# quocdat32461997/ggpm

Hardware: AMD Instinct MI355X
Metric: HierMPNEncoder fwd+bwd target row (SURVEY 8(d): encoder + KL heads + optimizer, tree fixed-point hint on; full depth loops in full_depth_loops, the full VAE fwd+bwd row in vae_step) of BASELINE's molecules/sec VAE fwd+bwd (hidden=300, depth=20, batch=32) (higher is better)
Workload: dtype f32

## Files before the change

### ggpm_amd/_lib.py

```python
from __future__ import annotations

import ctypes
import os
from ctypes import c_char_p, c_double, c_float, c_int, c_size_t, c_void_p, POINTER

from . import build as _build

_LIB = None

GGPM_OK, GGPM_ERR_ARG, GGPM_ERR_LAUNCH, GGPM_ERR_UNSUPPORTED, GGPM_ERR_WORKSPACE = range(5)

P = c_void_p
I = c_int
SIGNATURES = {
    "ggpm_version": (I, []),
    "ggpm_error_string": (c_char_p, [I]),
    "ggpm_padded_hidden": (I, [I]),
    "ggpm_padded_to_csr": (I, [P, I, I, P, P, P]),
    "ggpm_padded_to_csr_pair": (I, [P, I, I, P, P, P, I, I, P, P, P]),
    "ggpm_csr_transpose": (I, [P, P, I, I, P, P, P, P]),
    "ggpm_extract_column": (I, [P, I, I, I, P, P]),
    "ggpm_gemm_workspace_bytes": (c_size_t, [I, I, I]),
    "ggpm_gemm": (I, [I, I, I, I, I, P, I, P, I, P, I, I, P, I, I, I, P, c_size_t, P]),
    "ggpm_gemm_grouped": (I, [I, I, I, I, I, I, P, P]),
# ... 14 lines not shown
    "ggpm_gather_rows": (I, [P, I, P, I, I, P, I, I, I, P]),
    "ggpm_scatter_rows": (I, [P, I, P, I, I, P, I, I, P]),
    "ggpm_adam_step": (I, [P, P, P, P, c_size_t, c_float, c_float, c_float, c_float, c_float, I, P]),
    "ggpm_flat_sqnorm_workspace_bytes": (c_size_t, [c_size_t]),
    "ggpm_flat_sqnorm_partials": (I, [P, c_size_t, P, c_size_t, P]),
    "ggpm_flat_norm_finish": (I, [P, I, c_float, P, P]),
    "ggpm_adam_step_groups": (I, [P, P, P, P, c_size_t, P, I, P, I, P, I, c_float, P, I, P]),
    "ggpm_adam_step_ex": (I, [P, P, P, P, c_size_t, P, I, P, I, P, I, c_float, I, P, c_float, I, I, P, P, P, P]),
    "ggpm_flat_swap": (I, [P, P, c_size_t, P]),
    "ggpm_onehot": (I, [P, I, I, P, I, I, I, P]),
    "ggpm_embed_graph": (I, [P, I, P, I, I, I, I, P, I, P, I, P]),
    "ggpm_level_bf16_storage": (I, [I, I]),
    "ggpm_level_form_query": (I, [I, I, I, I, I, P, P]),
    "ggpm_level_q_part_bytes": (c_size_t, [I, I]),
    "ggpm_level_ksplit_q": (I, [I, I, I, I, P]),
    "ggpm_gru_backward_stashes": (I, [P, I, I, I, POINTER(c_void_p), POINTER(c_void_p)]),
    "ggpm_lstm_backward_stashes": (I, [P, I, I, I, POINTER(c_void_p), POINTER(c_void_p), POINTER(c_void_p)]),
    "ggpm_sum_slots": (I, [P, I, c_size_t, P, P]),
    "ggpm_gru_pack_floats": (c_size_t, [I]),
    "ggpm_gru_forward": (I, [I, I, I, P, P, P, P, I, P, I, P, P, I, P, P, P, P, P, P, P, P, P, P, I, P, P]),
    "ggpm_gru_backward_workspace_bytes": (c_size_t, [I, I, I]),
    "ggpm_gru_backward": (I, [I, I, I, P, P, I, P, I, P, I, P, P, P, P, P, P, P, P, P, P, P, P, P, P, P,
                              P, I, P, I, P, P, I, P, c_size_t, I, P, P]),
    "ggpm_gru_weight_grads": (I, [I, I, I, P, P, P, P, c_size_t, P, I, P, I, P, P, I, P, P]),
    "ggpm_gru_sparse_forward": (I, [I, I, I, P, P, P, P, P, P, I, P, I, P, P, I, P, P, P, P, P, P, P, P, P, P, I, P, P]),
    "ggpm_gru_sparse_backward": (I, [I, I, I, P, P, P, I, P, I, P, I, P, P, P, P, P, P, P, P, P, P, P, P, P, P, P, P,
                                     P, I, P, I, P, P, I, P, c_size_t, P, P]),
    "ggpm_weight_grads_stacked_workspace_bytes": (c_size_t, [I, I]),
    "ggpm_gru_weight_grads_stacked": (I, [I, I, I, P, P, P, P, P, P, P, I, P, I, P, P, I, P, c_size_t, P]),
    "ggpm_lstm_weight_grads_stacked": (I, [I, I, I, P, P, P, P, P, P, P, I, P, I, P, I, P, I, P, c_size_t, P]),
# ... 125 lines not shown
```

### ggpm_amd/csrc/encoder.hip

```cpp
#include "common.h"
#include "level_call.h"
#include <condition_variable>
#include <cstdlib>
#include <deque>
#include <functional>
#include <mutex>
#include <thread>

namespace {

struct Arena {
    char* base;
    size_t off;
    bool overflow;
    size_t cap;
    template <typename T>
    T* take(size_t n) {
        const size_t bytes = (n * sizeof(T) + 255) & ~(size_t)255;
        T* p = base ? reinterpret_cast<T*>(base + off) : nullptr;
        off += bytes;
        if (base && off > cap) overflow = true;
        return p;
    }
};
// ... 74 lines not shown
    const size_t slot = (size_t)E1 * Hp;
    L.X = A.take<float>(cell_gates(lstm).n * slot);
    L.Hs = A.take<float>((size_t)(depth + 1) * slot);
    L.Cs = lstm ? A.take<float>((size_t)(depth + 1) * slot) : nullptr;
    L.Qs = A.take<float>((size_t)depth * slot);
    L.St = A.take<float>((size_t)5 * depth * slot);
    L.wpack = A.take<float>(ggpm_level_pack_floats(lstm, H));
    L.nei = A.take<float>((size_t)N1 * Hp);
}

void take_q_part(Arena& A, const Dims& d, LevelSaved& L) {
    const ggpm_level_opts o = level_opts(d);
    L.qpart = nullptr; L.qpart_bytes = 0;
    if (!ggpm_level_ksplit_q(d.lstm, d.E1t, d.H, 0, &o)) return;
    L.qpart_bytes = ggpm_level_q_part_bytes(d.E1t, d.H);
    L.qpart = A.take<float>(L.qpart_bytes / sizeof(float));
}

void layout_saved(Arena& A, const Dims& d, Saved& s) {
    s.lv[0].hout = s.lv[1].hout = s.lv[2].hout = nullptr;
    take_csr(A, s.gpred, d.E1g, d.E1g, d.E1g * d.Kgb);
    take_csr(A, s.gagr, d.N1g, d.E1g, d.N1g * d.Kga);
    take_csr(A, s.tpred, d.E1t, d.E1t, d.E1t * d.Ktb);
    take_csr(A, s.tagr, d.N1t, d.E1t, d.N1t * d.Kta);
    take_csr(A, s.tcgr, d.N1t, d.N1g, d.N1t * d.Ktc);
    s.src = A.take<int32_t>(d.E1t); s.attr0 = A.take<int32_t>(d.E1t);
    s.motif_id = A.take<int32_t>(d.N1t); s.attach_id = A.take<int32_t>(d.N1t);
    const int nio = (d.E1t > d.N1t ? d.E1t : d.N1t) + 1;
    s.iota = A.take<int32_t>(nio > d.B + 1 ? nio : d.B + 1);
    auto take_index = [&](Csr& c, int rows, int ncols) {
// ... 4 lines not shown
    take_index(s.tsrc, d.E1t, d.N1t);
    take_index(s.root, d.B, d.N1t);
    take_index(s.motif, d.N1t, d.n_motif);
    take_index(s.attach, d.N1t, d.n_attach);
    s.hnode_a = A.take<float>((size_t)d.N1g * d.ld_n);
    s.hmess_a = A.take<float>((size_t)d.E1g * d.ld_m);
    take_level(A, s.lv[0], d.E1t, d.N1t, d.Hp, d.H, d.depthT, d.lstm);
    take_level(A, s.lv[1], d.E1t, d.N1t, d.Hp, d.H, d.depthT, d.lstm);
    take_level(A, s.lv[2], d.E1g, d.N1g, d.Hp, d.H, d.depthG, d.lstm);
    s.finput_i = A.take<float>((size_t)d.N1t * d.Hep); s.pooled = A.take<float>((size_t)d.N1t * d.Hp);
    s.hnode_i = A.take<float>((size_t)d.N1t * d.Hp); s.hmess_i = A.take<float>((size_t)d.E1t * d.ld_t);
    s.finput_t = A.take<float>((size_t)d.N1t * d.Hep);
    s.hnode_t = A.take<float>((size_t)d.N1t * d.Hp); s.hmess_t = A.take<float>((size_t)d.E1t * d.ld_t);
    s.f = A.take<float>((size_t)d.B * d.Hp); s.n = A.take<float>((size_t)d.B * d.Hp);
    for (int l = 0; l < 2; ++l) take_q_part(A, d, s.lv[l]);
    s.lv[2].qpart = nullptr; s.lv[2].qpart_bytes = 0;
}

void take_csr_fwd(Arena& A, Csr& c, int rows, int ncols, int cap) {
    c.rows = rows; c.ncols = ncols; c.cap = cap < 1 ? 1 : cap;
    c.rowptr = A.take<int32_t>(rows + 1);
    c.col = A.take<int32_t>(c.cap);
    c.rowptrT = c.colT = c.cursor = nullptr;
}

void layout_infer(Arena& A, const Dims& d, Saved& s) {
    s = Saved{};
    take_csr_fwd(A, s.gpred, d.E1g, d.E1g, d.E1g * d.Kgb);
    take_csr_fwd(A, s.gagr, d.N1g, d.E1g, d.N1g * d.Kga);
    take_csr_fwd(A, s.tpred, d.E1t, d.E1t, d.E1t * d.Ktb);
    take_csr_fwd(A, s.tagr, d.N1t, d.E1t, d.N1t * d.Kta);
// ... 9 lines not shown
    L.Qs = A.take<float>(2 * slot);
    L.Cs = d.lstm ? A.take<float>(2 * slot) : nullptr;
    L.hout = A.take<float>(slot);
    L.wpack = A.take<float>(ggpm_level_pack_floats(d.lstm, d.H));
    for (int l = 0; l < 3; ++l) {
        s.lv[l] = L;
        s.lv[l].nei = A.take<float>((size_t)(l == 2 ? d.N1g : d.N1t) * d.Hp);
    }
    s.finput_i = A.take<float>((size_t)d.N1t * d.Hep); s.pooled = A.take<float>((size_t)d.N1t * d.Hp);
    s.hnode_i = A.take<float>((size_t)d.N1t * d.Hp); s.hmess_i = A.take<float>((size_t)d.E1t * d.ld_t);
    s.finput_t = A.take<float>((size_t)d.N1t * d.Hep);
    s.hnode_t = A.take<float>((size_t)d.N1t * d.Hp); s.hmess_t = A.take<float>((size_t)d.E1t * d.ld_t);
    s.f = A.take<float>((size_t)d.B * d.Hp); s.n = A.take<float>((size_t)d.B * d.Hp);
    take_q_part(A, d, s.lv[0]);
    s.lv[1].qpart = s.lv[0].qpart; s.lv[1].qpart_bytes = s.lv[0].qpart_bytes;
}

__global__ void iota_k(int32_t* out, int n) {
    const int i = blockIdx.x * blockDim.x + threadIdx.x;
    if (i < n) out[i] = i;
}

enum { P_EC = 0, P_EI, P_WC, P_BC, P_WI, P_BI, P_WROOT, P_BROOT, P_LEVEL0 };
enum { L_WO = 0, L_BO, L_WZ, L_BZ, L_WR, L_UR, L_BU, L_WH, L_BH, L_COUNT };
enum { Q_WO = 0, Q_BO, Q_WI, Q_BI, Q_WOG, Q_BOG, Q_WU, Q_BU, Q_WF, Q_BF, Q_COUNT };
struct LevelSlots { int count, w[4], b[4], ur, bu, ld[4]; };
constexpr LevelSlots GRU_SLOTS = {L_COUNT, {L_WZ, L_WR, L_WH, -1}, {L_BZ, -1, L_BH, -1}, L_UR, L_BU, {}};
constexpr LevelSlots LSTM_SLOTS = {Q_COUNT, {Q_WI, Q_WOG, Q_WU, Q_WF}, {Q_BI, Q_BOG, Q_BU, Q_BF}, -1, -1, {}};
inline const LevelSlots& level_slots(bool lstm) { return lstm ? LSTM_SLOTS : GRU_SLOTS; }
inline int lwo(const Dims& d, int level) { return P_LEVEL0 + level * level_slots(d.lstm).count + L_WO; }
// ... 708 lines not shown
```

### ggpm_amd/csrc/level_host.h

```cpp
#pragma once
#include "tile_mma.h"
#include <cstdlib>
#include <type_traits>

namespace {

constexpr size_t GGPM_LDS_LIMIT = 160 * 1024;

template <typename K>
inline void set_lds(K kernel, size_t bytes) { ggpm_set_lds(kernel, bytes); }

inline bool env_no_fuse_b() { static const bool v = ggpm_dev_env("GGPM_NO_FUSE_B") != nullptr; return v; }
inline bool env_adebug() { static const bool v = ggpm_dev_env("GGPM_ADEBUG") != nullptr; return v; }

inline int pick_tg(int E1, int NT) {
    static const char* const tg_env = ggpm_dev_env("GGPM_TG");
    if (const char* e = tg_env) { int v = atoi(e); if (v >= 1 && v <= 64) return v; }
    static const char* const tg_small_env = ggpm_dev_env("GGPM_TG_SMALL");
    if (const char* e = tg_small_env) {
        int v = atoi(e);
        if (v >= 1 && v <= 64 && (E1 + 15) / 16 <= 64) return v < NT ? v : NT;
    }
    static const char* const tg_large_env = ggpm_dev_env("GGPM_TG_LARGE");
    if (const char* e = tg_large_env) {
// ... 25 lines not shown
template <class Cell>
inline LevelPlan level_plan(const ggpm_level_opts& o, int E1, int Hp, bool sparse) {
    LevelPlan p;
    p.tg = pick_tg(E1, Hp / 16);
    p.rt2 = Cell::use_rt2(o, E1, Hp, sparse);
    p.gm = gate_mode<Cell>(o, Hp, p.rt2, p.tg >= Hp / 16, sparse);
    return p;
}
constexpr int GGPM_KSPLIT_MAX_GROUPS = 5;
inline bool ksplit_q_form(const LevelPlan& p, int Hp) {
    static const bool on = [] { const char* e = ggpm_dev_env("GGPM_KSPLIT_Q"); return !e || atoi(e) != 0; }();
    const int groups = ggpm_ceil_div(Hp / 16, p.tg);
    return on && p.gm == 0 && !p.rt2 && groups >= 2 && groups <= GGPM_KSPLIT_MAX_GROUPS && p.tg <= 2 * GGPM_NWA;
}
inline size_t q_part_floats(int E1, int Hp, int tg) { return (size_t)2 * ggpm_ceil_div(Hp / 16, tg) * E1 * Hp; }

struct StepLds { int fuse; size_t a, b; };
inline StepLds step_lds(const StepNeed& need, int max_tiles, int Hp, int tg, bool rt2, int gm, bool may_fuse) {
    const int rows = rt2 ? 32 : 16, NT = Hp / 16;
    const bool split = gm == 2;
    const size_t fused = lds_bytes(need.fused, rows, Hp, split);
    StepLds p;
    p.fuse = (!rt2 && may_fuse && ggpm_ceil_div(NT, tg) == 1 && (!max_tiles || NT <= max_tiles) && fused <= GGPM_LDS_LIMIT &&
              !env_no_fuse_b()) ? 1 : 0;
    p.a = p.fuse ? fused : lds_bytes(need.a, rows, Hp, split);
    p.b = lds_bytes(need.b, rows, Hp, split);
    return p;
}
template <class Cell>
inline StepLds fwd_step(int Hp, int tg, bool rt2, int gm, bool with_b) {
// ... 160 lines not shown
```

### ggpm_amd/csrc/mpn_gru.hip

```cpp
#include "tile_mma.h"
#include "level_host.h"
#include "level_call.h"
#include <cstdlib>
#include <cstdio>

__global__ void ggpm_pack_weight_kernel(GgpmPackArgs a) {
    const int Hp = a.Hp, H = a.H, KC = Hp / 16;
    const int lane = threadIdx.x;
    const int kc = blockIdx.x, t = blockIdx.y, m = blockIdx.z;
    const float* __restrict__ W = a.W[m];
    const int ldw = a.ldw[m];
    const int out = 16 * t + (lane & 15);
    if (a.bf16 == 2) {
        const int KC32 = ggpm_kc32_dev(Hp);
        float x[8];
#pragma unroll
        for (int i = 0; i < 8; ++i) {
            const int k = 32 * kc + 8 * (lane >> 4) + i;
            x[i] = (out < H && k < H) ? (a.transpose ? W[(size_t)k * ldw + out] : W[(size_t)out * ldw + k]) : 0.f;
        }
        uint2 lo[3], hi[3];
        ggpm_split3(make_float4(x[0], x[1], x[2], x[3]), lo[0], lo[1], lo[2]);
        ggpm_split3(make_float4(x[4], x[5], x[6], x[7]), hi[0], hi[1], hi[2]);
        __bf16* dst = reinterpret_cast<__bf16*>(a.dst) + (size_t)m * 2 * ggpm_packed_matrix_floats(Hp, 2);
// ... 558 lines not shown
    const int row = r0 + (lane & 15);
    for (int tt = grp * a.tg + wave; tt < t_end; tt += GGPM_NWA) {
        const int c = 16 * tt + 4 * (lane >> 4);
        const float4 b = ggpm_ld4(a.bu + c);
        f32x4 head[4];
        ggpm_slice_head(a.Ur, KC, tt, 0, min(NT, a.tg), lane, head);
        float4 q = ggpm_zero4();
        for (int gi = 0; gi < a.groups; ++gi) {
            const int k0 = gi * a.tg, k1 = min(NT, k0 + a.tg);
            f32x4 acc = {0.f, 0.f, 0.f, 0.f};
            ggpm_wave_gemm_slice(Th, LD, a.Ur, KC, tt, k0, k1, gi + 1 < a.groups ? tt : -1, k1, min(NT, k1 + a.tg), lane, acc, head);
            q = gi == 0 ? ggpm_f4(acc) + b : q + ggpm_f4(acc);
        }
        if (row < a.E1) ggpm_st4(a.Qnew + (size_t)row * Hp + c, q);
    }
}

template <int GM, int RTT, bool ST16 = false>
__global__ void GGPM_A_BOUNDS gru_fwd_b(GruFwdArgs a) {
    constexpr int ROWS = RTT * 16;
    constexpr bool BF16 = GM == 1, SPLIT = GM == 2;
    static_assert(!SPLIT || RTT == 1, "split operands: one row tile per workgroup");
    extern __shared__ __attribute__((aligned(16))) float lds[];
    const int Hp = a.Hp, LD = Hp + 4, KC = Hp / 16, NT = Hp / 16;
    float* Th = lds;
    const int LDH = ggpm_split_ldh(Hp), PLANE = ROWS * LDH, KC32 = ggpm_kc32_dev(Hp);
    __bf16* Ih = reinterpret_cast<__bf16*>(lds);
    const int lane = threadIdx.x & 63;
    const int wave = __builtin_amdgcn_readfirstlane(threadIdx.x >> 6);
    const int r0 = blockIdx.x * ROWS;
// ... 381 lines not shown
        if (lds_tiles(2, Hp, 32) > GGPM_LDS_LIMIT) return false;
        return mode == 2 || o.prefer_narrow || ggpm_ceil_div(E1, 16) >= GGPM_RT2_MIN_ROW_TILES;
    }
    static bool mode2_fits(int Hp) { return lds_tiles(1, Hp) + 2 * ggpm_split_image_bytes(16, Hp) <= GGPM_LDS_LIMIT; }
    static bool shape_ok(int, int Hp) { return lds_tiles(2, Hp) <= GGPM_LDS_LIMIT; }
};

inline unsigned long long* adebug_stamps(unsigned long long*& buf) {
    if (!env_adebug()) return nullptr;
    if (!buf) (void)hipMalloc(&buf, 64);
    return buf;
}

inline dim3 ks_grid(const GruFwdArgs& a) { return dim3(8 * ggpm_ceil_div(ggpm_ceil_div(a.E1, 16), 8) * a.groups); }

void launch_fwd(GruFwdArgs a, bool rt2, bool stash, bool with_b, bool ks, double flops1, hipStream_t s) {
    const StepLds step = fwd_step<GruCell>(a.Hp, a.tg, rt2, a.bf16, with_b);
    a.fuse_b = step.fuse;
    if (ks) {
        static unsigned long long* ks_dbg_buf = nullptr;
        static int ks_dbg_count = 0;
        a.dbg = adebug_stamps(ks_dbg_buf);
        ggpm_timing_begin(GruCell::timing_base, s, ((a.Qpart_out ? 1 : 0) + (a.h0_zero ? 0 : GruCell::gate_products)) * flops1);
        {
            auto kernel = stash ? gru_fwd_a_ks<true> : gru_fwd_a_ks<false>;
            set_lds(kernel, step.a);
            kernel<<<ks_grid(a), GGPM_NWA * 64, step.a, s>>>(a);
        }
        ggpm_timing_end(GruCell::timing_base, s);
        if (a.dbg && a.Qpart_in && a.Qpart_out && (++ks_dbg_count % 97) == 0) {
            unsigned long long h[8];
// ... 75 lines not shown
int ggpm_gru_level_form(int E1, int H, int sparse, int training, const ggpm_level_opts& o, ggpm_level_form* out) {
    return level_form<GruCell>(E1, H, sparse, training, o, out);
}

extern "C" size_t ggpm_level_q_part_bytes(int E1, int H) {
    if (E1 <= 0 || H <= 0) return 0;
    const int Hp = ggpm_padded_hidden(H);
    return q_part_floats(E1, Hp, pick_tg(E1, Hp / 16)) * sizeof(float);
}
extern "C" int ggpm_level_ksplit_q(int lstm, int E1, int H, int sparse, const ggpm_level_opts* opts) {
    if (lstm || sparse || E1 <= 0 || H <= 0) return 0;
    const int Hp = ggpm_padded_hidden(H);
    if (!GruCell::shape_ok(E1, Hp)) return 0;
    return ksplit_q_form(level_plan<GruCell>(ggpm_opts_or_default(opts), E1, Hp, false), Hp) ? 1 : 0;
}

namespace {
__global__ void sparse_init_state(const float* __restrict__ h_in, const unsigned char* __restrict__ frozen,
                                  float* __restrict__ H0, int Hp) {
    const int c = blockIdx.x * blockDim.x + threadIdx.x;
    const int r = blockIdx.y;
    if (c >= Hp) return;
    H0[(size_t)r * Hp + c] = frozen[r] ? h_in[(size_t)r * Hp + c] : 0.f;
}
}

int gru_forward_impl(const LevelCall& c, int save_for_backward, const ggpm_level_opts& o, ggpm_stream_t stream) {
    GGPM_CLEAR_STALE_ERROR();
    const int E1 = c.rows, H = c.H, depth = c.depth;
    float *Hs = c.Hs, *Qs = c.Qs, *wpack = c.wpack;
    const unsigned char* frozen = c.frozen;
    bool ok = E1 > 0 && H > 0 && depth > 0 && c.bu && c.pred_rowptr && c.pred_col && Hs && Qs && wpack;
    for (int k = 0; k < 3; ++k) ok = ok && c.X[k] && c.W[k];
    for (int k = 0; k < 5; ++k) ok = ok && (c.St[k] || !save_for_backward);
    if (!ok) return GGPM_ERR_ARG;
    const int Hp = ggpm_padded_hidden(H);
    if (!GruCell::shape_ok(E1, Hp)) return GGPM_ERR_UNSUPPORTED;
    hipStream_t s = (hipStream_t)stream;
    const size_t slot = (size_t)E1 * Hp;
    const LevelPlan plan = level_plan<GruCell>(o, E1, Hp, frozen != nullptr);
    const bool rt2 = plan.rt2;
    const int bf16 = plan.gm;
    const bool ks = o.q_part && !frozen && ksplit_q_form(plan, Hp);
    const size_t qblock = q_part_floats(E1, Hp, plan.tg) / 2;
    if (ks && o.q_part_bytes < 2 * qblock * sizeof(float)) return GGPM_ERR_WORKSPACE;
    const size_t mstep = ggpm_packed_matrix_floats(Hp, bf16);
    float* pWz = wpack; float* pWh = wpack + mstep; float* pUr = wpack + 2 * mstep;
    float* pbu = wpack + 3 * ggpm_packed_matrix_slot(Hp);
    {
        GgpmPackArgs pk = {};
        pk.W[0] = c.W[0]; pk.ldw[0] = c.ldw[0]; pk.W[1] = c.W[2]; pk.ldw[1] = c.ldw[2]; pk.W[2] = c.W[1]; pk.ldw[2] = c.ldw[1];
        pk.H = H; pk.Hp = Hp; pk.transpose = 0; pk.dst = wpack; pk.bias = c.bu; pk.bias_out = pbu; pk.bf16 = bf16;
        if (!o.weights_packed) ggpm_launch_pack(pk, 3, s);
    }
    dim3 ig(ggpm_ceil_div(Hp, 256), E1);
    const int tg0 = plan.tg;
    const bool gathered = o.gather_h && o.gather_idx && frozen;
    if (frozen) {
        if (c.h_in != Hs && !gathered) sparse_init_state<<<ig, 256, 0, s>>>(c.h_in, frozen, Hs, Hp);
        GruFwdArgs a0 = {};
// ... 42 lines not shown
            }
            a.S = a.G = a.Z = a.M = a.R = nullptr;
        } else {
            a.Hprev = Hs + (size_t)((t - 1) & 1) * slot; a.Hnew = Hs + (size_t)(t & 1) * slot;
            a.Qprev = Qs + (size_t)((t - 1) & 1) * slot; a.Qnew = Qs + (size_t)(t & 1) * slot;
            a.S = a.G = a.Z = a.M = a.R = nullptr;
        }
        if (ks) {
            a.groups = ggpm_ceil_div(Hp / 16, tg);
            if (t < run_depth) a.Qpart_out = o.q_part + (size_t)(t & 1) * qblock;
            if (t > 1) {
                a.Qpart_in = o.q_part + (size_t)((t - 1) & 1) * qblock;
                a.Qsum = save_for_backward ? const_cast<float*>(a.Qprev) : nullptr;
            }
        }
        launch_fwd(a, rt2, stash, t < depth, ks, flops1, s);
    }
    GGPM_CHECK_LAUNCH();
    return GGPM_OK;
}

#define GRU_FORWARD_OPERANDS(c) \
    c.rows = E1; c.H = H; c.depth = depth; \
    c.X[0] = Xz; c.X[1] = Xr; c.X[2] = Xh; \
    c.W[0] = Wz_h; c.ldw[0] = ld_wz; c.W[1] = Ur; c.ldw[1] = ld_ur; c.W[2] = Wh_h; c.ldw[2] = ld_wh; c.bu = bu; \
    c.pred_rowptr = pred_rowptr; c.pred_col = pred_col; \
    c.Hs = Hs; c.Qs = Qs; c.St[0] = Ss; c.St[1] = Gs; c.St[2] = Zs; c.St[3] = Ms; c.St[4] = Rs; c.wpack = wpack;
extern "C" int ggpm_gru_forward(int E1, int H, int depth, const float* Xz, const float* Xr, const float* Xh,
                                const float* Wz_h, int ld_wz, const float* Ur, int ld_ur, const float* bu,
                                const float* Wh_h, int ld_wh, const int32_t* pred_rowptr,
                                const int32_t* pred_col, float* Hs, float* Qs, float* Ss, float* Gs, float* Zs,
// ... 307 lines not shown
```

### ggpm_amd/csrc/tile_mma.h

```cpp
#pragma once
#include "common.h"
#include <type_traits>

constexpr int GGPM_NW = 4;
#ifndef GGPM_NWA_VALUE
#define GGPM_NWA_VALUE 16
#endif
constexpr int GGPM_NWA = GGPM_NWA_VALUE;
#if GGPM_NWA_VALUE == 16
#define GGPM_A_BOUNDS __launch_bounds__(1024)
#else
#define GGPM_A_BOUNDS __launch_bounds__(GGPM_NWA_VALUE * 64, 4)
#endif
constexpr int GGPM_PF = 4;
#ifndef GGPM_PF3
#define GGPM_PF3 3
#endif
#ifndef GGPM_CHAIN_MAX
#define GGPM_CHAIN_MAX 3
#endif
#ifndef GGPM_PF1
#define GGPM_PF1 GGPM_PF
#endif
template <int NOPS> struct GgpmPf { static constexpr int value = NOPS >= 3 ? GGPM_PF3 : (NOPS == 1 ? GGPM_PF1 : GGPM_PF); };
// ... 212 lines not shown
        const float x2 = __builtin_bit_cast(float, r1b[e] & 0xffff0000u);
        r2b[e] = __builtin_bit_cast(unsigned, r1 - x2);
    }
    p1 = make_uint2(b1[0] | (b1[1] << 16), b1[2] | (b1[3] << 16));
    p2 = make_uint2(__builtin_amdgcn_perm(r1b[1], r1b[0], 0x07060302u), __builtin_amdgcn_perm(r1b[3], r1b[2], 0x07060302u));
    p3 = make_uint2(__builtin_amdgcn_perm(r2b[1], r2b[0], 0x07060302u), __builtin_amdgcn_perm(r2b[3], r2b[2], 0x07060302u));
}

__device__ __forceinline__ void ggpm_split_store(__bf16* img, int PLANE, int LDH, int lr, int c, float4 x) {
    uint2 p1, p2, p3;
    ggpm_split3(x, p1, p2, p3);
    __bf16* d = img + lr * LDH + c;
    *reinterpret_cast<uint2*>(d) = p1;
    *reinterpret_cast<uint2*>(d + PLANE) = p2;
    *reinterpret_cast<uint2*>(d + 2 * PLANE) = p3;
}

__device__ __forceinline__ void ggpm_split_init(__bf16* img0, int nimg, int rows, int Hp) {
    const int LDH = Hp + 8, IMG = 3 * rows * LDH + 8;
    for (int it = threadIdx.x; it < nimg * (3 * rows + 1); it += blockDim.x) {
        const int im = it / (3 * rows + 1), r = it - im * (3 * rows + 1);
        __bf16* d = img0 + (size_t)im * IMG + (r < 3 * rows ? r * LDH + Hp : 3 * rows * LDH);
        *reinterpret_cast<uint4*>(d) = make_uint4(0u, 0u, 0u, 0u);
    }
}

template <int ROWS>
__device__ __forceinline__ void ggpm_load_rows_to_lds_split(const float* __restrict__ src, int r0, int rows, int Hp,
                                                            __bf16* img, int PLANE, int LDH) {
    const int q = Hp >> 2;
// ... 42 lines not shown
__device__ __forceinline__ void ggpm_split_ring_prefetch(const float* const (&wps_f32)[NOPS], int KC32, int t, int lane,
                                                         GgpmSplitRing<NOPS>& ring) {
    constexpr int PF = GgpmSplitPf<NOPS>::value;
#pragma unroll
    for (int d = 0; d < PF; ++d) {
        const int kk = min(d, KC32 - 1);
#pragma unroll
        for (int o = 0; o < NOPS; ++o)
#pragma unroll
            for (int p = 0; p < 3; ++p)
                ring.r[d][o][p] = *reinterpret_cast<const bf16x8*>(reinterpret_cast<const __bf16*>(wps_f32[o]) +
                                                                   ggpm_pack_index_split(t, kk, KC32, p, lane));
    }
}

template <int NOPS, bool SHARED = false, bool SUM = false>
__device__ __forceinline__ void ggpm_wave_gemm_split(const __bf16* const (&imgs)[NOPS], int PLANE, int LDH,
                                                     const float* const (&wps_f32)[NOPS], int KC32, int t, int t_next,
                                                     int lane, f32x4 (&acc)[NOPS][1], GgpmSplitRing<NOPS>& ring) {
    constexpr int PF = GgpmSplitPf<NOPS>::value;
    constexpr int NACC = SUM ? 1 : NOPS;
#ifdef GGPM_ABL_LDS_BROADCAST
    const int boff = 8 * (lane >> 4);
#else
    const int boff = (lane & 15) * LDH + 8 * (lane >> 4);
#endif
    const bool chain = t_next >= 0 && (KC32 % PF) == 0;
    const __bf16* wp[NOPS];
    const __bf16* wn[NOPS];
#pragma unroll
    for (int o = 0; o < NOPS; ++o) {
        wp[o] = reinterpret_cast<const __bf16*>(wps_f32[o]) + ggpm_pack_index_split(t, 0, KC32, 0, lane);
        wn[o] = reinterpret_cast<const __bf16*>(wps_f32[o]) + ggpm_pack_index_split(chain ? t_next : t, 0, KC32, 0, lane);
    }
    f32x4 lo[NACC];
#pragma unroll
    for (int o = 0; o < NACC; ++o) lo[o] = f32x4{0.f, 0.f, 0.f, 0.f};
    for (int kc = 0; kc < KC32; kc += PF) {
#pragma unroll
        for (int d = 0; d < PF; ++d) {
            if (kc + d < KC32) {
                const int kq = kc + d + PF;
                const bool over = kq >= KC32;
                const int kn = over ? (chain ? kq - KC32 : KC32 - 1) : kq;
                bf16x8 b[3];
#pragma unroll
                for (int o = 0; o < NOPS; ++o) {
                    if (o == 0 || !SHARED) {
#pragma unroll
                        for (int p = 0; p < 3; ++p)
                            b[p] = *reinterpret_cast<const bf16x8*>(imgs[o] + p * PLANE + boff + 32 * (kc + d));
                    }
                    constexpr int Z = 0;
                    f32x4& hi_ = acc[SUM ? Z : o][0];
                    f32x4& lo_ = lo[SUM ? Z : o];
                    lo_ = __builtin_amdgcn_mfma_f32_16x16x32_bf16(ring.r[d][o][2], b[0], lo_, 0, 0, 0);
                    lo_ = __builtin_amdgcn_mfma_f32_16x16x32_bf16(ring.r[d][o][0], b[2], lo_, 0, 0, 0);
                    hi_ = __builtin_amdgcn_mfma_f32_16x16x32_bf16(ring.r[d][o][0], b[0], hi_, 0, 0, 0);
                    lo_ = __builtin_amdgcn_mfma_f32_16x16x32_bf16(ring.r[d][o][1], b[1], lo_, 0, 0, 0);
                    lo_ = __builtin_amdgcn_mfma_f32_16x16x32_bf16(ring.r[d][o][1], b[0], lo_, 0, 0, 0);
                    lo_ = __builtin_amdgcn_mfma_f32_16x16x32_bf16(ring.r[d][o][0], b[1], lo_, 0, 0, 0);
                }
                __builtin_amdgcn_sched_barrier(0);
#ifndef GGPM_ABL_NOLOAD_SPLIT
#pragma unroll
                for (int o = 0; o < NOPS; ++o)
#pragma unroll
                    for (int p = 0; p < 3; ++p)
                        ring.r[d][o][p] = *reinterpret_cast<const bf16x8*>((over && chain ? wn[o] : wp[o]) +
                                                                           ((size_t)kn * 3 + p) * 512);
#else
                (void)kn; (void)over;
#endif
                __builtin_amdgcn_sched_barrier(0);
            }
        }
    }
#pragma unroll
    for (int o = 0; o < NACC; ++o) acc[o][0] = acc[o][0] + lo[o];
    if (t_next >= 0 && !chain) ggpm_split_ring_prefetch<NOPS>(wps_f32, KC32, t_next, lane, ring);
}

template <int NOPS, int RT>
__device__ __forceinline__ void ggpm_zero_acc(f32x4 (&acc)[NOPS][RT]) {
#pragma unroll
    for (int o = 0; o < NOPS; ++o)
#pragma unroll
        for (int r = 0; r < RT; ++r) acc[o][r] = f32x4{0.f, 0.f, 0.f, 0.f};
}

__device__ __forceinline__ float4 ggpm_f4(f32x4 v) { return make_float4(v[0], v[1], v[2], v[3]); }

__device__ __forceinline__ float4 ggpm_bf16x4_to_f4(uint2 v) {
    return make_float4(__builtin_bit_cast(float, v.x << 16), __builtin_bit_cast(float, v.x & 0xffff0000u),
                       __builtin_bit_cast(float, v.y << 16), __builtin_bit_cast(float, v.y & 0xffff0000u));
// ... 107 lines not shown
```

### include/ggpm_hip.h

```cpp
#ifndef GGPM_HIP_H
#define GGPM_HIP_H

#include <stddef.h>
#include <stdint.h>

#ifdef __cplusplus
extern "C" {
#endif

typedef void* ggpm_stream_t;

enum {
    GGPM_OK = 0,
    GGPM_ERR_ARG = 1,
    GGPM_ERR_LAUNCH = 2,
    GGPM_ERR_UNSUPPORTED = 3,
    GGPM_ERR_WORKSPACE = 4
};

enum { GGPM_ACT_NONE = 0, GGPM_ACT_RELU = 1, GGPM_ACT_TANH = 2, GGPM_ACT_SIGMOID = 3 };

int ggpm_version(void);
const char* ggpm_error_string(int code);
int ggpm_padded_hidden(int H);
// ... 157 lines not shown
    float* scatter_c;
    const int32_t* scatter_idx;
    int skip_x_sums;
    int run_depth;
    int lo;
    int skip_bias_u;
    int skip_sparse_wgrads;
    float* h_out;
    float* c_out;
    int fixed_slot;
    float* q_part;
    size_t q_part_bytes;
} ggpm_level_opts;
size_t ggpm_level_q_part_bytes(int E1, int H);
int ggpm_level_ksplit_q(int lstm, int E1, int H, int sparse, const ggpm_level_opts* opts);

typedef struct ggpm_level_form {
    int Hp, tiles;
    int tg, groups;
    int rt2, gate_mode, st16;
    int fuse_fwd, fuse_bwd;
    size_t lds_fwd_a, lds_fwd_b, lds_bwd_a, lds_bwd_b;
} ggpm_level_form;
int ggpm_level_form_query(int lstm, int E1, int H, int sparse, int training, const ggpm_level_opts* opts,
                          ggpm_level_form* out);

size_t ggpm_gru_pack_floats(int H);
int ggpm_gru_forward(int E1, int H, int depth, const float* Xz, const float* Xr, const float* Xh,
                     const float* Wz_h, int ld_wz, const float* Ur, int ld_ur, const float* bu,
                     const float* Wh_h, int ld_wh, const int32_t* pred_rowptr, const int32_t* pred_col,
// ... 333 lines not shown
```

Before: 12460.

## Add two-tile k-split GRU forward kernel for atom-level message passing

Adds a new GRU forward kernel for the atom (graph) level that processes 32 rows per workgroup as two 16-row tiles and splits the next step's reset-gate product Ur·h across two column groups. Partial sums go to a double-buffered q_part workspace that the next step consumes. The atom level now receives a q_part allocation, where it previously had none. This aims to cut redundant weight loads and to overlap the next step's reset-gate GEMM with the current step. It adds extra workspace, a second partial-sum read per gather, and debug timestamp plumbing that can occasionally synchronize the stream.

```diff
diff --git a/ggpm_amd/_lib.py b/ggpm_amd/_lib.py
--- a/ggpm_amd/_lib.py
+++ b/ggpm_amd/_lib.py
@@ -52,6 +52,8 @@
     "ggpm_level_form_query": (I, [I, I, I, I, I, P, P]),
     "ggpm_level_q_part_bytes": (c_size_t, [I, I]),
     "ggpm_level_ksplit_q": (I, [I, I, I, I, P]),
+    "ggpm_level_two_tile_q_bytes": (c_size_t, [I, I]),
+    "ggpm_level_two_tile_q": (I, [I, I, I, I, P]),
     "ggpm_gru_backward_stashes": (I, [P, I, I, I, POINTER(c_void_p), POINTER(c_void_p)]),
     "ggpm_lstm_backward_stashes": (I, [P, I, I, I, POINTER(c_void_p), POINTER(c_void_p), POINTER(c_void_p)]),
     "ggpm_sum_slots": (I, [P, I, c_size_t, P, P]),
diff --git a/ggpm_amd/csrc/encoder.hip b/ggpm_amd/csrc/encoder.hip
--- a/ggpm_amd/csrc/encoder.hip
+++ b/ggpm_amd/csrc/encoder.hip
@@ -112,6 +112,14 @@
     L.qpart = nullptr; L.qpart_bytes = 0;
     if (!ggpm_level_ksplit_q(d.lstm, d.E1t, d.H, 0, &o)) return;
     L.qpart_bytes = ggpm_level_q_part_bytes(d.E1t, d.H);
+    L.qpart = A.take<float>(L.qpart_bytes / sizeof(float));
+}
+
+void take_q_part_atom(Arena& A, const Dims& d, LevelSaved& L) {
+    const ggpm_level_opts o = level_opts(d);
+    L.qpart = nullptr; L.qpart_bytes = 0;
+    if (!ggpm_level_two_tile_q(d.lstm, d.E1g, d.H, 0, &o)) return;
+    L.qpart_bytes = ggpm_level_two_tile_q_bytes(d.E1g, d.H);
     L.qpart = A.take<float>(L.qpart_bytes / sizeof(float));
 }
 
@@ -146,7 +154,7 @@
     s.hnode_t = A.take<float>((size_t)d.N1t * d.Hp); s.hmess_t = A.take<float>((size_t)d.E1t * d.ld_t);
     s.f = A.take<float>((size_t)d.B * d.Hp); s.n = A.take<float>((size_t)d.B * d.Hp);
     for (int l = 0; l < 2; ++l) take_q_part(A, d, s.lv[l]);
-    s.lv[2].qpart = nullptr; s.lv[2].qpart_bytes = 0;
+    take_q_part_atom(A, d, s.lv[2]);
 }
 
 void take_csr_fwd(Arena& A, Csr& c, int rows, int ncols, int cap) {
@@ -186,6 +194,7 @@
     s.f = A.take<float>((size_t)d.B * d.Hp); s.n = A.take<float>((size_t)d.B * d.Hp);
     take_q_part(A, d, s.lv[0]);
     s.lv[1].qpart = s.lv[0].qpart; s.lv[1].qpart_bytes = s.lv[0].qpart_bytes;
+    take_q_part_atom(A, d, s.lv[2]);
 }
 
 __global__ void iota_k(int32_t* out, int n) {
diff --git a/ggpm_amd/csrc/level_host.h b/ggpm_amd/csrc/level_host.h
--- a/ggpm_amd/csrc/level_host.h
+++ b/ggpm_amd/csrc/level_host.h
@@ -63,6 +63,20 @@
     return on && p.gm == 0 && !p.rt2 && groups >= 2 && groups <= GGPM_KSPLIT_MAX_GROUPS && p.tg <= 2 * GGPM_NWA;
 }
 inline size_t q_part_floats(int E1, int Hp, int tg) { return (size_t)2 * ggpm_ceil_div(Hp / 16, tg) * E1 * Hp; }
+
+inline int two_tile_tg(int NT) { return 2 * ggpm_ceil_div(NT, 4); }
+inline size_t two_tile_lds(int Hp) {
+    return 2 * ggpm_split_image_bytes(32, Hp) + ggpm_split_image_bytes(32, 16 * two_tile_tg(Hp / 16));
+}
+inline dim3 tt_grid(int E1) { return dim3(8 * ggpm_ceil_div(ggpm_ceil_div(E1, 32), 8) * 2); }
+inline bool two_tile_q_form(const LevelPlan& p, int E1, int Hp) {
+    static const bool on = [] { const char* e = ggpm_dev_env("GGPM_KSPLIT_Q"); return !e || atoi(e) != 0; }();
+    const int NT = Hp / 16, tg = two_tile_tg(NT);
+    const bool waves_ok = tg <= 2 * GGPM_SLICE_MAXC && tg + (NT > GGPM_NWA ? NT - GGPM_NWA : 0) < GGPM_NWA;
+    return on && p.gm == 2 && !p.rt2 && p.tg >= NT && tg < NT && waves_ok && Hp <= 320 &&
+           2 * ggpm_ceil_div(E1, 32) <= 256 && two_tile_lds(Hp) <= GGPM_LDS_LIMIT;
+}
+inline size_t two_tile_q_floats(int E1, int Hp) { return (size_t)2 * 2 * E1 * Hp; }
 
 struct StepLds { int fuse; size_t a, b; };
 inline StepLds step_lds(const StepNeed& need, int max_tiles, int Hp, int tg, bool rt2, int gm, bool may_fuse) {
diff --git a/ggpm_amd/csrc/mpn_gru.hip b/ggpm_amd/csrc/mpn_gru.hip
--- a/ggpm_amd/csrc/mpn_gru.hip
+++ b/ggpm_amd/csrc/mpn_gru.hip
@@ -596,6 +596,224 @@
         }
         if (row < a.E1) ggpm_st4(a.Qnew + (size_t)row * Hp + c, q);
     }
+}
+
+template <bool STASH>
+__global__ void GGPM_A_BOUNDS gru_fwd_a_tt(GruFwdArgs a) {
+    extern __shared__ __attribute__((aligned(16))) float lds[];
+    const int Hp = a.Hp, NT = Hp / 16;
+    const int LDH = ggpm_split_ldh(Hp), PLANE = 32 * LDH, KC32 = ggpm_kc32_dev(Hp);
+    const int IMG = ggpm_split_image_halves(32, Hp);
+    const int lane = threadIdx.x & 63;
+    const int wave = __builtin_amdgcn_readfirstlane(threadIdx.x >> 6);
+    const int rblock = ((int)(blockIdx.x >> 3) >> 1) * 8 + (int)(blockIdx.x & 7);
+    if (rblock * 32 >= a.E1) return;
+    const int r0 = rblock * 32;
+    const int grp = (int)(blockIdx.x >> 3) & 1;
+    const int k0 = grp * a.tg, k1 = min(NT, k0 + a.tg);
+    const int WS = 16 * (k1 - k0), LDHS = WS + 8, PLANES = 32 * LDHS;
+    __bf16* Is = reinterpret_cast<__bf16*>(lds);
+    __bf16* Ig = Is + IMG;
+    __bf16* Ih = Ig + IMG;
+    ggpm_split_init(Is, 2, 32, Hp);
+    ggpm_split_init(Ih, 1, 32, WS);
+    const size_t pslot = (size_t)a.E1 * Hp;
+    const bool dbg_on = a.dbg && rblock == 1 && grp == 0 && threadIdx.x == 0;
+    if (dbg_on) a.dbg[0] = wall_clock64();
+
+    {
+        int row[2];
+        GgpmRowList rl[2];
+#pragma unroll
+        for (int i = 0; i < 2; ++i) {
+            row[i] = r0 + wave + 16 * i;
+            if (a.h0_zero) { rl[i].lo = 0; rl[i].n = 0; } else rl[i] = ggpm_row_list(a.rowptr, row[i], a.E1);
+        }
+        const int c = lane * 4, tc = 256 + lane;
+        const bool on = c < Hp, ton = tc < Hp;
+        const int cs = on ? c : 0, tcs = ton ? tc : 0;
+        float4 s[2], g[2], rc[2], xr[2];
+        float s1[2], g1[2], rc1[2], xr1[2];
+#pragma unroll
+        for (int i = 0; i < 2; ++i) {
+            const size_t rowo = (size_t)(row[i] < a.E1 ? row[i] : 0) * Hp;
+            s[i] = ggpm_zero4(); g[i] = ggpm_zero4(); rc[i] = ggpm_zero4();
+            s1[i] = g1[i] = rc1[i] = 0.f;
+            xr[i] = ggpm_ld4(a.Xr + rowo + cs);
+            xr1[i] = a.Xr[rowo + tcs];
+        }
+        const int nmax = max(rl[0].n, rl[1].n);
+        for (int base = 0; base < nmax; base += 64) {
+            int chunk[2], m[2];
+#pragma unroll
+            for (int i = 0; i < 2; ++i) {
+                chunk[i] = ggpm_list_chunk(a.col, rl[i], base, lane);
+                m[i] = max(0, min(64, rl[i].n - base));
+            }
+            const int mm = max(m[0], m[1]);
+            for (int j = 0; j < mm; j += GGPM_GATHER_U) {
+                float4 h[GGPM_GATHER_U][2], qp[GGPM_GATHER_U][2][2];
+                float h1[GGPM_GATHER_U][2], qp1[GGPM_GATHER_U][2][2];
+#pragma unroll
+                for (int u = 0; u < GGPM_GATHER_U; ++u)
+#pragma unroll
+                    for (int i = 0; i < 2; ++i) {
+                        if (j + u >= m[i]) continue;
+                        const size_t p = (size_t)__builtin_amdgcn_readlane(chunk[i], j + u) * Hp;
+                        h[u][i] = ggpm_ld4(a.Hprev + p + cs);
+                        h1[u][i] = a.Hprev[p + tcs];
+#pragma unroll
+                        for (int gi = 0; gi < 2; ++gi) {
+                            qp[u][i][gi] = ggpm_ld4(a.Qpart_in + gi * pslot + p + cs);
+                            qp1[u][i][gi] = a.Qpart_in[gi * pslot + p + tcs];
+                        }
+                    }
+#pragma unroll
+                for (int u = 0; u < GGPM_GATHER_U; ++u)
+#pragma unroll
+                    for (int i = 0; i < 2; ++i) {
+                        if (j + u >= m[i]) continue;
+                        const float4 r = ggpm_fsigmoid4<false>(xr[i] + (qp[u][i][0] + qp[u][i][1]));
+                        const float4 rh = r * h[u][i];
+                        s[i] = s[i] + h[u][i];
+                        g[i] = g[i] + rh;
+                        rc[i] = rc[i] + rh * one_minus(r);
+                        const float r1 = ggpm_fsigmoid<false>(xr1[i] + (qp1[u][i][0] + qp1[u][i][1])), rh1 = r1 * h1[u][i];
+                        s1[i] = s1[i] + h1[u][i];
+                        g1[i] = g1[i] + rh1;
+                        rc1[i] = rc1[i] + rh1 * (1.f - r1);
+                    }
+            }
+        }
+#pragma unroll
+        for (int i = 0; i < 2; ++i) {
+            const int lr = wave + 16 * i;
+            if (on) {
+                ggpm_split_store(Is, PLANE, LDH, lr, c, s[i]);
+                ggpm_split_store(Ig, PLANE, LDH, lr, c, g[i]);
+                if (STASH && row[i] < a.E1 && (c >> 4) / a.tg == grp) {
+                    const size_t o = (size_t)row[i] * Hp + c;
+                    ggpm_st4(a.S + o, s[i]); ggpm_st4(a.G + o, g[i]); ggpm_st4(a.R + o, rc[i]);
+                }
+            }
+            if (ton) {
+                ggpm_split_store1(Is, PLANE, LDH, lr, tc, s1[i]);
+                ggpm_split_store1(Ig, PLANE, LDH, lr, tc, g1[i]);
+                if (STASH && row[i] < a.E1 && (tc >> 4) / a.tg == grp) {
+                    const size_t o = (size_t)row[i] * Hp + tc;
+                    a.S[o] = s1[i]; a.G[o] = g1[i]; a.R[o] = rc1[i];
+                }
+            }
+        }
+    }
+    if (dbg_on) a.dbg[1] = wall_clock64();
+
+    const int t = k0 + wave;
+    const bool p2_gemm = !a.h0_zero;
+    const float* const wps2[2] = {a.Wz, a.Wh};
+    GgpmSplitRing<2> sring2;
+    if (p2_gemm && t < k1) ggpm_split_ring_prefetch<2>(wps2, KC32, t, lane, sring2);
+    ggpm_lds_barrier();
+    if (dbg_on) a.dbg[2] = wall_clock64();
+
+    const int lr = lane & 15;
+    const int kc0 = k0 >> 1, kc1 = (k1 + 1) >> 1;
+    const int t3b = GGPM_NWA + (GGPM_NWA - 1 - wave);
+    const bool p3 = a.Qpart_out != nullptr;
+    GgpmSliceFrags uf;
+    float4 bias = ggpm_zero4();
+    auto p3_loads = [&](int tt) {
+        ggpm_split_slice_load(a.Ur, KC32, tt, kc0, kc1, lane, uf);
+        if (grp == 0) bias = ggpm_ld4(a.bu + 16 * tt + 4 * (lane >> 4));
+    };
+    if (t >= k1) {
+        const int w0 = k1 - k0, nw = min(GGPM_NWA, 2 * GGPM_NWA - NT) - w0;
+        if (a.Qsum && a.Qpart_in && wave < w0 + nw) {
+            const int n4 = 4 * (k1 - k0), total = 32 * n4;
+            for (int i0 = (wave - w0) * 64 + lane; i0 < total; i0 += 4 * nw * 64) {
+                float4 q0[4], q1[4];
+                size_t o[4];
+                bool ok[4];
+#pragma unroll
+                for (int u = 0; u < 4; ++u) {
+                    const int i = i0 + u * nw * 64, orow = r0 + i / n4;
+                    ok[u] = i < total && orow < a.E1;
+                    o[u] = ok[u] ? (size_t)orow * Hp + 16 * k0 + 4 * (i % n4) : 0;
+                    q0[u] = ggpm_ld4(a.Qpart_in + o[u]);
+                    q1[u] = ggpm_ld4(a.Qpart_in + pslot + o[u]);
+                }
+#pragma unroll
+                for (int u = 0; u < 4; ++u)
+                    if (ok[u]) ggpm_st4(a.Qsum + o[u], q0[u] + q1[u]);
+            }
+        }
+        if (p3 && wave < NT) p3_loads(wave);
+    } else {
+        const int c = 16 * t + 4 * (lane >> 4);
+        float4 xz[2], xh[2];
+        auto load_inputs = [&]() {
+#pragma unroll
+            for (int r = 0; r < 2; ++r) {
+                const int row = r0 + 16 * r + lr;
+                const size_t o = (size_t)(row < a.E1 ? row : 0) * Hp + c;
+                xz[r] = ggpm_ld4(a.Xz + o);
+                xh[r] = ggpm_ld4(a.Xh + o);
+            }
+        };
+        f32x4 acc[2][2];
+        ggpm_zero_acc<2, 2>(acc);
+        if (p2_gemm) {
+            const __bf16* const imgs[2] = {Is, Ig};
+            ggpm_wave_gemm_split<2, false, false, 2>(imgs, PLANE, LDH, wps2, KC32, t, -1, lane, acc, sring2);
+        }
+        load_inputs();
+        if (dbg_on) a.dbg[3] = wall_clock64();
+        float4 h[2], z[2], m[2];
+#pragma unroll
+        for (int r = 0; r < 2; ++r) {
+            const int lrow = 16 * r + lr, row = r0 + lrow;
+            h[r] = ggpm_zero4(); z[r] = ggpm_zero4(); m[r] = ggpm_zero4();
+            if (row < a.E1 && row != 0) {
+                const float4 s = a.h0_zero ? ggpm_zero4() : ggpm_split_load(Is, PLANE, LDH, lrow, c);
+                const float4 pz = ggpm_f4(acc[0][r]) + xz[r], pm = ggpm_f4(acc[1][r]) + xh[r];
+                z[r] = ggpm_sigmoid4(pz);
+                m[r] = make_float4(tanhf(pm.x), tanhf(pm.y), tanhf(pm.z), tanhf(pm.w));
+                h[r] = make_float4((1.f - z[r].x) * s.x + z[r].x * m[r].x, (1.f - z[r].y) * s.y + z[r].y * m[r].y,
+                                   (1.f - z[r].z) * s.z + z[r].z * m[r].z, (1.f - z[r].w) * s.w + z[r].w * m[r].w);
+            }
+            if (p3) ggpm_split_store(Ih, PLANES, LDHS, lrow, c - 16 * k0, h[r]);
+        }
+        if (p3 && wave < NT) p3_loads(wave);
+#pragma unroll
+        for (int r = 0; r < 2; ++r) {
+            const int row = r0 + 16 * r + lr;
+            if (row >= a.E1) continue;
+            const size_t o = (size_t)row * Hp + c;
+            ggpm_st4(a.Hnew + o, h[r]);
+            if (STASH) {
+                ggpm_st4(a.Z + o, z[r]);
+                ggpm_st4(a.M + o, m[r]);
+            }
+        }
+    }
+    if (dbg_on) a.dbg[4] = wall_clock64();
+    if (!p3) return;
+
+    ggpm_lds_barrier();
+    float* const part = a.Qpart_out + (size_t)grp * pslot;
+    for (int tt = wave; tt < NT; tt = (tt == wave ? t3b : NT)) {
+        const int c = 16 * tt + 4 * (lane >> 4);
+        f32x4 acc[2] = {f32x4{0.f, 0.f, 0.f, 0.f}, f32x4{0.f, 0.f, 0.f, 0.f}};
+        ggpm_wave_gemm_split_slice<2>(Ih, PLANES, LDHS, kc1 - kc0, lane, acc, uf);
+        const float4 b = bias;
+        if (tt == wave && t3b < NT) p3_loads(t3b);
+#pragma unroll
+        for (int r = 0; r < 2; ++r) {
+            const int row = r0 + 16 * r + lr;
+            if (row < a.E1) ggpm_st4(part + (size_t)row * Hp + c, grp == 0 ? ggpm_f4(acc[r]) + b : ggpm_f4(acc[r]));
+        }
+    }
+    if (dbg_on) a.dbg[7] = wall_clock64();
 }
 
 template <int GM, int RTT, bool ST16 = false>
@@ -1007,7 +1225,29 @@
 
 inline dim3 ks_grid(const GruFwdArgs& a) { return dim3(8 * ggpm_ceil_div(ggpm_ceil_div(a.E1, 16), 8) * a.groups); }
 
-void launch_fwd(GruFwdArgs a, bool rt2, bool stash, bool with_b, bool ks, double flops1, hipStream_t s) {
+void launch_fwd(GruFwdArgs a, bool rt2, bool stash, bool with_b, bool ks, bool tt, double flops1, hipStream_t s) {
+    if (tt) {
+        static unsigned long long* tt_dbg_buf = nullptr;
+        static int tt_dbg_count = 0;
+        a.dbg = adebug_stamps(tt_dbg_buf);
+        const size_t lds = two_tile_lds(a.Hp);
+        ggpm_timing_begin(GruCell::timing_base, s, ((a.Qpart_out ? 1 : 0) + (a.h0_zero ? 0 : GruCell::gate_products)) * flops1);
+        {
+            auto kernel = stash ? gru_fwd_a_tt<true> : gru_fwd_a_tt<false>;
+            set_lds(kernel, lds);
+            kernel<<<tt_grid(a.E1), GGPM_NWA * 64, lds, s>>>(a);
+        }
+        ggpm_timing_end(GruCell::timing_base, s);
+        if (a.dbg && a.Qpart_in && a.Qpart_out && (++tt_dbg_count % 97) == 0) {
+            unsigned long long h[8];
+            (void)hipStreamSynchronize(s);
+            (void)hipMemcpy(h, a.dbg, sizeof(h), hipMemcpyDeviceToHost);
+            fprintf(stderr, "[adebug two-tile E1=%d wgs=%d] gather %.2f wait %.2f P2 %.2f epilogue %.2f partial q' %.2f us\n", a.E1,
+                    (int)tt_grid(a.E1).x, (h[1] - h[0]) * 0.01, (h[2] - h[1]) * 0.01, (h[3] - h[2]) * 0.01, (h[4] - h[3]) * 0.01,
+                    (h[7] - h[4]) * 0.01);
+        }
+        return;
+    }
     const StepLds step = fwd_step<GruCell>(a.Hp, a.tg, rt2, a.bf16, with_b);
     a.fuse_b = step.fuse;
     if (ks) {
@@ -1113,6 +1353,16 @@
     if (!GruCell::shape_ok(E1, Hp)) return 0;
     return ksplit_q_form(level_plan<GruCell>(ggpm_opts_or_default(opts), E1, Hp, false), Hp) ? 1 : 0;
 }
+extern "C" size_t ggpm_level_two_tile_q_bytes(int E1, int H) {
+    if (E1 <= 0 || H <= 0) return 0;
+    return two_tile_q_floats(E1, ggpm_padded_hidden(H)) * sizeof(float);
+}
+extern "C" int ggpm_level_two_tile_q(int lstm, int E1, int H, int sparse, const ggpm_level_opts* opts) {
+    if (lstm || sparse || E1 <= 0 || H <= 0) return 0;
+    const int Hp = ggpm_padded_hidden(H);
+    if (!GruCell::shape_ok(E1, Hp)) return 0;
+    return two_tile_q_form(level_plan<GruCell>(ggpm_opts_or_default(opts), E1, Hp, false), E1, Hp) ? 1 : 0;
+}
 
 namespace {
 __global__ void sparse_init_state(const float* __restrict__ h_in, const unsigned char* __restrict__ frozen,
@@ -1143,6 +1393,9 @@
     const bool ks = o.q_part && !frozen && ksplit_q_form(plan, Hp);
     const size_t qblock = q_part_floats(E1, Hp, plan.tg) / 2;
     if (ks && o.q_part_bytes < 2 * qblock * sizeof(float)) return GGPM_ERR_WORKSPACE;
+    const bool tt = o.q_part && !frozen && !(o.run_depth > 0 && o.run_depth < depth) && o.fixed_slot <= 0 && two_tile_q_form(plan, E1, Hp);
+    const size_t tblock = two_tile_q_floats(E1, Hp) / 2;
+    if (tt && o.q_part_bytes < 2 * tblock * sizeof(float)) return GGPM_ERR_WORKSPACE;
     const size_t mstep = ggpm_packed_matrix_floats(Hp, bf16);
     float* pWz = wpack; float* pWh = wpack + mstep; float* pUr = wpack + 2 * mstep;
     float* pbu = wpack + 3 * ggpm_packed_matrix_slot(Hp);
@@ -1215,7 +1468,16 @@
                 a.Qsum = save_for_backward ? const_cast<float*>(a.Qprev) : nullptr;
             }
         }
-        launch_fwd(a, rt2, stash, t < depth, ks, flops1, s);
+        if (tt) {
+            a.groups = 2;
+            a.tg = two_tile_tg(Hp / 16);
+            if (t < run_depth) a.Qpart_out = o.q_part + (size_t)(t & 1) * tblock;
+            if (t > 1) {
+                a.Qpart_in = o.q_part + (size_t)((t - 1) & 1) * tblock;
+                a.Qsum = save_for_backward ? const_cast<float*>(a.Qprev) : nullptr;
+            }
+        }
+        launch_fwd(a, rt2, stash, t < depth, ks, tt, flops1, s);
     }
     GGPM_CHECK_LAUNCH();
     return GGPM_OK;
diff --git a/ggpm_amd/csrc/tile_mma.h b/ggpm_amd/csrc/tile_mma.h
--- a/ggpm_amd/csrc/tile_mma.h
+++ b/ggpm_amd/csrc/tile_mma.h
@@ -250,6 +250,25 @@
     *reinterpret_cast<uint2*>(d) = p1;
     *reinterpret_cast<uint2*>(d + PLANE) = p2;
     *reinterpret_cast<uint2*>(d + 2 * PLANE) = p3;
+}
+
+__device__ __forceinline__ void ggpm_split_store1(__bf16* img, int PLANE, int LDH, int lr, int c, float x) {
+    const unsigned b1 = (unsigned)__builtin_bit_cast(unsigned short, (__bf16)x);
+    const float r1 = x - __builtin_bit_cast(float, b1 << 16);
+    const unsigned r1b = __builtin_bit_cast(unsigned, r1);
+    const unsigned r2b = __builtin_bit_cast(unsigned, r1 - __builtin_bit_cast(float, r1b & 0xffff0000u));
+    unsigned short* d = reinterpret_cast<unsigned short*>(img + lr * LDH + c);
+    d[0] = (unsigned short)b1;
+    d[PLANE] = (unsigned short)(r1b >> 16);
+    d[2 * PLANE] = (unsigned short)(r2b >> 16);
+}
+__device__ __forceinline__ float4 ggpm_split_load(const __bf16* img, int PLANE, int LDH, int lr, int c) {
+    const __bf16* d = img + lr * LDH + c;
+    const uint2 p1 = *reinterpret_cast<const uint2*>(d), p2 = *reinterpret_cast<const uint2*>(d + PLANE),
+                p3 = *reinterpret_cast<const uint2*>(d + 2 * PLANE);
+    auto f = [](unsigned w, int hi) { return __builtin_bit_cast(float, hi ? (w & 0xffff0000u) : (w << 16)); };
+    return make_float4((f(p3.x, 0) + f(p2.x, 0)) + f(p1.x, 0), (f(p3.x, 1) + f(p2.x, 1)) + f(p1.x, 1),
+                       (f(p3.y, 0) + f(p2.y, 0)) + f(p1.y, 0), (f(p3.y, 1) + f(p2.y, 1)) + f(p1.y, 1));
 }
 
 __device__ __forceinline__ void ggpm_split_init(__bf16* img0, int nimg, int rows, int Hp) {
@@ -322,10 +341,10 @@
     }
 }
 
-template <int NOPS, bool SHARED = false, bool SUM = false>
+template <int NOPS, bool SHARED = false, bool SUM = false, int RT = 1>
 __device__ __forceinline__ void ggpm_wave_gemm_split(const __bf16* const (&imgs)[NOPS], int PLANE, int LDH,
                                                      const float* const (&wps_f32)[NOPS], int KC32, int t, int t_next,
-                                                     int lane, f32x4 (&acc)[NOPS][1], GgpmSplitRing<NOPS>& ring) {
+                                                     int lane, f32x4 (&acc)[NOPS][RT], GgpmSplitRing<NOPS>& ring) {
     constexpr int PF = GgpmSplitPf<NOPS>::value;
     constexpr int NACC = SUM ? 1 : NOPS;
 #ifdef GGPM_ABL_LDS_BROADCAST
@@ -341,9 +360,11 @@
         wp[o] = reinterpret_cast<const __bf16*>(wps_f32[o]) + ggpm_pack_index_split(t, 0, KC32, 0, lane);
         wn[o] = reinterpret_cast<const __bf16*>(wps_f32[o]) + ggpm_pack_index_split(chain ? t_next : t, 0, KC32, 0, lane);
     }
-    f32x4 lo[NACC];
-#pragma unroll
-    for (int o = 0; o < NACC; ++o) lo[o] = f32x4{0.f, 0.f, 0.f, 0.f};
+    f32x4 lo[NACC][RT];
+#pragma unroll
+    for (int o = 0; o < NACC; ++o)
+#pragma unroll
+        for (int r = 0; r < RT; ++r) lo[o][r] = f32x4{0.f, 0.f, 0.f, 0.f};
     for (int kc = 0; kc < KC32; kc += PF) {
 #pragma unroll
         for (int d = 0; d < PF; ++d) {
@@ -351,23 +372,28 @@
                 const int kq = kc + d + PF;
                 const bool over = kq >= KC32;
                 const int kn = over ? (chain ? kq - KC32 : KC32 - 1) : kq;
-                bf16x8 b[3];
+                bf16x8 b[RT][3];
 #pragma unroll
                 for (int o = 0; o < NOPS; ++o) {
                     if (o == 0 || !SHARED) {
 #pragma unroll
-                        for (int p = 0; p < 3; ++p)
-                            b[p] = *reinterpret_cast<const bf16x8*>(imgs[o] + p * PLANE + boff + 32 * (kc + d));
+                        for (int r = 0; r < RT; ++r)
+#pragma unroll
+                            for (int p = 0; p < 3; ++p)
+                                b[r][p] = *reinterpret_cast<const bf16x8*>(imgs[o] + p * PLANE + r * 16 * LDH + boff + 32 * (kc + d));
                     }
                     constexpr int Z = 0;
-                    f32x4& hi_ = acc[SUM ? Z : o][0];
-                    f32x4& lo_ = lo[SUM ? Z : o];
-                    lo_ = __builtin_amdgcn_mfma_f32_16x16x32_bf16(ring.r[d][o][2], b[0], lo_, 0, 0, 0);
-                    lo_ = __builtin_amdgcn_mfma_f32_16x16x32_bf16(ring.r[d][o][0], b[2], lo_, 0, 0, 0);
-                    hi_ = __builtin_amdgcn_mfma_f32_16x16x32_bf16(ring.r[d][o][0], b[0], hi_, 0, 0, 0);
-                    lo_ = __builtin_amdgcn_mfma_f32_16x16x32_bf16(ring.r[d][o][1], b[1], lo_, 0, 0, 0);
-                    lo_ = __builtin_amdgcn_mfma_f32_16x16x32_bf16(ring.r[d][o][1], b[0], lo_, 0, 0, 0);
-                    lo_ = __builtin_amdgcn_mfma_f32_16x16x32_bf16(ring.r[d][o][0], b[1], lo_, 0, 0, 0);
+#pragma unroll
+                    for (int r = 0; r < RT; ++r) {
+                        f32x4& hi_ = acc[SUM ? Z : o][r];
+                        f32x4& lo_ = lo[SUM ? Z : o][r];
+                        lo_ = __builtin_amdgcn_mfma_f32_16x16x32_bf16(ring.r[d][o][2], b[r][0], lo_, 0, 0, 0);
+                        lo_ = __builtin_amdgcn_mfma_f32_16x16x32_bf16(ring.r[d][o][0], b[r][2], lo_, 0, 0, 0);
+                        hi_ = __builtin_amdgcn_mfma_f32_16x16x32_bf16(ring.r[d][o][0], b[r][0], hi_, 0, 0, 0);
+                        lo_ = __builtin_amdgcn_mfma_f32_16x16x32_bf16(ring.r[d][o][1], b[r][1], lo_, 0, 0, 0);
+                        lo_ = __builtin_amdgcn_mfma_f32_16x16x32_bf16(ring.r[d][o][1], b[r][0], lo_, 0, 0, 0);
+                        lo_ = __builtin_amdgcn_mfma_f32_16x16x32_bf16(ring.r[d][o][0], b[r][1], lo_, 0, 0, 0);
+                    }
                 }
                 __builtin_amdgcn_sched_barrier(0);
 #ifndef GGPM_ABL_NOLOAD_SPLIT
@@ -385,8 +411,51 @@
         }
     }
 #pragma unroll
-    for (int o = 0; o < NACC; ++o) acc[o][0] = acc[o][0] + lo[o];
+    for (int o = 0; o < NACC; ++o)
+#pragma unroll
+        for (int r = 0; r < RT; ++r) acc[o][r] = acc[o][r] + lo[o][r];
     if (t_next >= 0 && !chain) ggpm_split_ring_prefetch<NOPS>(wps_f32, KC32, t_next, lane, ring);
+}
+
+constexpr int GGPM_SLICE_MAXC = 5;
+struct GgpmSliceFrags { bf16x8 r[GGPM_SLICE_MAXC][3]; };
+__device__ __forceinline__ void ggpm_split_slice_load(const float* wp_f32, int KC32, int t, int kc0, int kc1, int lane,
+                                                      GgpmSliceFrags& f) {
+#pragma unroll
+    for (int d = 0; d < GGPM_SLICE_MAXC; ++d)
+        if (kc0 + d < kc1) {
+#pragma unroll
+            for (int p = 0; p < 3; ++p)
+                f.r[d][p] = *reinterpret_cast<const bf16x8*>(reinterpret_cast<const __bf16*>(wp_f32) +
+                                                             ggpm_pack_index_split(t, kc0 + d, KC32, p, lane));
+        }
+}
+template <int RT>
+__device__ __forceinline__ void ggpm_wave_gemm_split_slice(const __bf16* img, int PLANE, int LDH, int nchunks, int lane,
+                                                           f32x4 (&acc)[RT], const GgpmSliceFrags& f) {
+    const int boff = (lane & 15) * LDH + 8 * (lane >> 4);
+    f32x4 lo[RT];
+#pragma unroll
+    for (int r = 0; r < RT; ++r) lo[r] = f32x4{0.f, 0.f, 0.f, 0.f};
+#pragma unroll
+    for (int d = 0; d < GGPM_SLICE_MAXC; ++d) {
+        if (d < nchunks) {
+#pragma unroll
+            for (int r = 0; r < RT; ++r) {
+                bf16x8 b[3];
+#pragma unroll
+                for (int p = 0; p < 3; ++p) b[p] = *reinterpret_cast<const bf16x8*>(img + p * PLANE + r * 16 * LDH + boff + 32 * d);
+                lo[r] = __builtin_amdgcn_mfma_f32_16x16x32_bf16(f.r[d][2], b[0], lo[r], 0, 0, 0);
+                lo[r] = __builtin_amdgcn_mfma_f32_16x16x32_bf16(f.r[d][0], b[2], lo[r], 0, 0, 0);
+                acc[r] = __builtin_amdgcn_mfma_f32_16x16x32_bf16(f.r[d][0], b[0], acc[r], 0, 0, 0);
+                lo[r] = __builtin_amdgcn_mfma_f32_16x16x32_bf16(f.r[d][1], b[1], lo[r], 0, 0, 0);
+                lo[r] = __builtin_amdgcn_mfma_f32_16x16x32_bf16(f.r[d][1], b[0], lo[r], 0, 0, 0);
+                lo[r] = __builtin_amdgcn_mfma_f32_16x16x32_bf16(f.r[d][0], b[1], lo[r], 0, 0, 0);
+            }
+        }
+    }
+#pragma unroll
+    for (int r = 0; r < RT; ++r) acc[r] = acc[r] + lo[r];
 }
 
 template <int NOPS, int RT>
diff --git a/include/ggpm_hip.h b/include/ggpm_hip.h
--- a/include/ggpm_hip.h
+++ b/include/ggpm_hip.h
@@ -195,6 +195,8 @@
 } ggpm_level_opts;
 size_t ggpm_level_q_part_bytes(int E1, int H);
 int ggpm_level_ksplit_q(int lstm, int E1, int H, int sparse, const ggpm_level_opts* opts);
+size_t ggpm_level_two_tile_q_bytes(int E1, int H);
+int ggpm_level_two_tile_q(int lstm, int E1, int H, int sparse, const ggpm_level_opts* opts);
 
 typedef struct ggpm_level_form {
     int Hp, tiles;
```

After: 12580 (median of 6 runs). Within noise of the previous version (+1.0%).
